# 3DGenomes/TADpole

Measured on NVIDIA B200. Metric: tadpole_calls_per_sec, higher is better.
Workload: dtype f64

## Files before the change

### tadpole_b200/csrc/api.cu

```cuda
#include "common.cuh"
#include <stdarg.h>
#include <algorithm>
#include <mutex>
#include <numeric>
#include <unordered_map>

int tp_sweep_device(tp_ctx *ctx, int min_clusters, int cand_begin, int cand_stride, int *ncand_out);
int tp_ch_device(tp_ctx *ctx, int min_clusters, int ncand, int ld_chs);

static thread_local char g_err[1024] = "";

void tp_set_error(const char *fmt, ...) {
    va_list ap;
    va_start(ap, fmt);
    vsnprintf(g_err, sizeof(g_err), fmt, ap);
    va_end(ap);
}

extern "C" const char *tp_last_error(void) { return g_err; }
extern "C" int tp_version(void) { return 103; }

int tp_pin_reserve(tp_ctx *ctx, size_t bytes) {
    if (bytes <= ctx->pin_cap) return TP_OK;
    if (ctx->pin) cudaFreeHost(ctx->pin);
// ... 57 lines not shown
    }
    TP_ARG(device >= 0 && device < ndev, "tp_ctx_create: device index out of range");
    TP_CUDA(cudaSetDevice(device));
    cudaDeviceProp prop;
    TP_CUDA(cudaGetDeviceProperties(&prop, device));
    if (prop.major < 10) {
        tp_set_error("tp_ctx_create: device %d is sm_%d%d; this library is built for sm_100a (B200) only",
                     device, prop.major, prop.minor);
        return TP_ERR_CUDA;
    }
    tp_ctx *ctx = new tp_ctx();
    ctx->device = device;
    ctx->sm_count = prop.multiProcessorCount;
    ctx->max_smem_optin = (int)prop.sharedMemPerBlockOptin;
    TP_CUDA(cudaStreamCreateWithFlags(&ctx->stream, cudaStreamNonBlocking));
    for (int i = 0; i < EV_COUNT; i++) TP_CUDA(cudaEventCreate(&ctx->ev[i]));
    TP_CUDA(cudaEventCreateWithFlags(&ctx->sync_ev, cudaEventBlockingSync | cudaEventDisableTiming));
    TP_TRY(tp_pin_reserve(ctx, 1 << 16));
    TP_TRY(tp_flags_reset(ctx));
    if (const char *tune = getenv("TADPOLE_TUNE")) {
        std::string t(tune);
        size_t pos = 0;
        while (pos < t.size()) {
            size_t end = t.find(',', pos);
            if (end == std::string::npos) end = t.size();
            const std::string item = t.substr(pos, end - pos);
            pos = end + 1;
            if (item.empty()) continue;
            const size_t eq = item.find('=');
            char *endp = nullptr;
            const double v = eq == std::string::npos ? 0.0 : strtod(item.c_str() + eq + 1, &endp);
            if (eq == std::string::npos || eq == 0 || endp == item.c_str() + eq + 1 || *endp) {
                tp_set_error("tp_ctx_create: TADPOLE_TUNE item '%s' is not key=number", item.c_str());
                tp_ctx_destroy(ctx);
                return TP_ERR_ARG;
            }
            if (tp_ctx_set(ctx, item.substr(0, eq).c_str(), v) != TP_OK) { tp_ctx_destroy(ctx); return TP_ERR_ARG; }
        }
    }
    *out = ctx;
    return TP_OK;
}

extern "C" int tp_ctx_destroy(tp_ctx *ctx) {
    if (!ctx) return TP_OK;
    tp_pool_destroy(ctx);
    tp_group_destroy(ctx);
    cudaSetDevice(ctx->device);
    tp_stream_sync(ctx);
    DevBuf *bufs[] = {&ctx->raw_own, &ctx->rowmean, &ctx->ranks, &ctx->flags, &ctx->qtmp, &ctx->keep, &ctx->X, &ctx->C,
                      &ctx->colstat, &ctx->scores, &ctx->M, &ctx->Y0, &ctx->Y1, &ctx->Y2, &ctx->W, &ctx->G, &ctx->T,
                      &ctx->Q, &ctx->Jw, &ctx->Jv, &ctx->Jt, &ctx->small1, &ctx->small2, &ctx->part, &ctx->resid,
                      &ctx->P, &ctx->Qp, &ctx->d0, &ctx->seqdist, &ctx->order, &ctx->ncl, &ctx->chs, &ctx->bsbuf,
                      &ctx->links, &ctx->harm, &ctx->status, &ctx->islices, &ctx->ioA, &ctx->ioB, &ctx->ioscale, &ctx->lx, &ctx->ly, &ctx->dout, &ctx->dhash, &ctx->lhash,
                      &ctx->itext, &ctx->icounts, &ctx->irows, &ctx->islow, &ctx->icoo, &ctx->raw_next};
    for (DevBuf *b : bufs) b->release();
    tp_comm_destroy_all(ctx);
    for (int i = 0; i < EV_COUNT; i++) if (ctx->ev[i]) cudaEventDestroy(ctx->ev[i]);
    for (cudaEvent_t e : ctx->prof_ev) cudaEventDestroy(e);
    if (ctx->sync_ev) cudaEventDestroy(ctx->sync_ev);
    if (ctx->staged_ev) cudaEventDestroy(ctx->staged_ev);
    for (tp_ctx::UploadLane &ln : ctx->lanes) {
        if (ln.st) { cudaStreamSynchronize(ln.st); cudaStreamDestroy(ln.st); }
        if (ln.done) cudaEventDestroy(ln.done);
        for (int b = 0; b < 2; b++) { if (ln.pin[b]) cudaFreeHost(ln.pin[b]); if (ln.ev[b]) cudaEventDestroy(ln.ev[b]); }
    }
    if (ctx->copy_stream) { cudaStreamSynchronize(ctx->copy_stream); cudaStreamDestroy(ctx->copy_stream); }
    for (int b = 0; b < 2; b++) {
        if (ctx->ipin[b]) cudaFreeHost(ctx->ipin[b]);
        if (ctx->ipin_ev[b]) cudaEventDestroy(ctx->ipin_ev[b]);
    }
    if (ctx->pin) cudaFreeHost(ctx->pin);
    if (ctx->pin_flags) cudaFreeHost(ctx->pin_flags);
    if (ctx->stream) cudaStreamDestroy(ctx->stream);
    delete ctx;
    return TP_OK;
}

extern "C" int tp_ctx_sync(tp_ctx *ctx) {
    TP_ARG(ctx, "tp_ctx_sync: null context");
    for (int r = tp_group_size(ctx) - 1; r >= 0; r--) {
        tp_ctx *m = tp_group_member(ctx, r);
        TP_CUDA(cudaSetDevice(m->device));
        TP_CUDA(tp_stream_sync(m));
    }
    return TP_OK;
}

extern "C" void *tp_ctx_stream(tp_ctx *ctx) { return ctx ? (void *)ctx->stream : nullptr; }
extern "C" long long tp_ctx_launches(tp_ctx *ctx) { return ctx ? ctx->launches : 0; }

extern "C" int tp_ctx_set(tp_ctx *ctx, const char *key, double value) {
    TP_ARG(ctx && key, "tp_ctx_set: null argument");
    if (tp_group_dispatch(ctx)) {
        for (int r = 1; r < tp_group_size(ctx); r++) {
            tp_ctx *m = tp_group_member(ctx, r);
            TpGroup *g = m->group;
            m->group = nullptr;
            const int rc = tp_ctx_set(m, key, value);
            m->group = g;
            TP_TRY(rc);
        }
    }
    std::string k(key);
    if (k == "pca_block") ctx->pca_block = (int)value;
    else if (k == "pca_tol") ctx->pca_tol = value;
    else if (k == "pca_maxit") ctx->pca_maxit = (int)value;
// ... 612 lines not shown
```

### tadpole_b200/csrc/common.cuh

```cuda
#pragma once
#include <cuda_runtime.h>
#include <stdint.h>
#include <stdio.h>
#include <string.h>
#include <math.h>
#include <string>
#include <vector>
#include <functional>
#include "../../include/tadpole_b200.h"

void tp_set_error(const char *fmt, ...);

#define TP_CUDA(call)                                                                     \
    do {                                                                                  \
        cudaError_t e_ = (call);                                                          \
        if (e_ != cudaSuccess) {                                                          \
            tp_set_error("%s:%d: %s -> %s", __FILE__, __LINE__, #call, cudaGetErrorString(e_)); \
            return TP_ERR_CUDA;                                                           \
        }                                                                                 \
    } while (0)

#define TP_TRY(call)                   \
    do {                               \
        int rc_ = (call);              \
// ... 62 lines not shown
    int comm_cur = -1;
    bool comm_grouped = false;
    int last_sweep_ranks = 1;
    int dist_min_n = 4096;
    int igemm_min_n = 1024;
    int iop_min_n = 1024;
    int sync_blocking = 0;
    cudaEvent_t sync_ev = nullptr;
    int shard_sym = 1;
    int mgram_min_n = 1024;
    int iop_final_min_n = 1024;
    int iop_final = 8;
    int io_bn32 = -1;
    double iop_switch = 1e-3;

    int pca_block = 0;
    double pca_tol = 1e-12;
    int pca_maxit = 16;
    int pca_inner = 4;
    int jacobi_direct_max = 512;
    int level_cap = 256;

    DevBuf itext, icounts, irows, islow, icoo;
    void *ipin[2] = {nullptr, nullptr};
    cudaEvent_t ipin_ev[2] = {nullptr, nullptr};
    struct UploadLane { cudaStream_t st = nullptr; void *pin[2] = {nullptr, nullptr}; cudaEvent_t ev[2] = {nullptr, nullptr}; cudaEvent_t done = nullptr; };
    std::vector<UploadLane> lanes;
    int upload_lanes = 4;
    int ingested_n = 0;
    double ingest_stats[4] = {};

    DevBuf raw_own;
    DevBuf raw_next;
    cudaStream_t copy_stream = nullptr;
    cudaEvent_t staged_ev = nullptr;
    const double *staged_mat = nullptr;
    int staged_n = 0, staged_colmajor = 0;
    std::function<void()> after_filter, after_pca;
    const double *raw = nullptr;
    int n = 0;
    int colmajor = 0;
    DevBuf rowmean, ranks, flags, qtmp, keep;
    int nf = 0, ldx = 0;
    DevBuf ioA, ioB, ioscale;
    int io_n = 0;
    bool io_cmax_clean = false;
    DevBuf X, C, colstat, islices;
    bool have_X = false, have_C = false;
    int k = 0, ldk = 0;
    int k_full = 0;
    DevBuf scores, M, Y0, Y1, Y2, W, G, T, Q, Jw, Jv, Jt, small1, small2, part, resid;
    DevBuf status;
    bool have_scores = false;
    DevBuf P, Qp, d0, seqdist, order, ncl, chs, bsbuf, links, harm;
    int ld_chs = 0;
    int last_maxlev = 0;
    std::vector<double> sweep_scores;
    bool have_sweep = false;
    DevBuf lx, ly, dout, dhash, lhash;
    void *pin = nullptr;
    size_t pin_cap = 0;
    int *pin_flags = nullptr;

    double timing[10] = {};
    long lowprec_applications = 0;

    bool prof = false;
    std::vector<cudaEvent_t> prof_ev;
    std::vector<int> prof_cls;
    size_t prof_used = 0;
    double prof_gemm_flop = 0.0;
    double prof_imma_ops = 0.0;
};

enum { PC_ROWMEAN = 0, PC_COMPACT, PC_GEMM, PC_JACOBI, PC_SWEEP, PC_CH, PC_DIFFT, PC_SPARE, PC_CHOL, PC_IGEMM, PC_COMM, PC_SPARE3, PC_ISLICE, PC_SPARE4, PC_SPARE5, PC_SPARE6, PC_COUNT };
void tp_prof_begin(tp_ctx *ctx, int cls);
void tp_prof_end(tp_ctx *ctx);

cudaError_t tp_optin_smem_fn(const void *kernel, const tp_ctx *ctx);
template <class K> static inline cudaError_t tp_optin_smem(K kernel, const tp_ctx *ctx) {
    return tp_optin_smem_fn((const void *)kernel, ctx);
}
int tp_pin_reserve(tp_ctx *ctx, size_t bytes);
cudaError_t tp_stream_sync(tp_ctx *ctx);

static inline int tp_nranks(const tp_ctx *ctx) { return ctx->comm_cur < 0 ? 1 : ctx->comm[ctx->comm_cur].nranks; }
static inline int tp_rank(const tp_ctx *ctx) { return ctx->comm_cur < 0 ? 0 : ctx->comm[ctx->comm_cur].rank; }
struct TpRows { int rpr, r0, r1, padded; };
static inline TpRows tp_rows(const tp_ctx *ctx, int n) {
    const int R = tp_nranks(ctx), rank = tp_rank(ctx);
    TpRows t;
    t.rpr = round_up((n + R - 1) / R, 64);
    t.r0 = rank * t.rpr < n ? rank * t.rpr : n;
    t.r1 = t.r0 + t.rpr < n ? t.r0 + t.rpr : n;
    t.padded = R * t.rpr;
    return t;
}
static inline bool tp_row_sharded(const tp_ctx *ctx, int n) { return tp_nranks(ctx) > 1 && n >= ctx->dist_min_n; }

struct SymShard { int R, rpr; };
__host__ __device__ inline bool ss_need(int i, int j, SymShard s) {
    const int a = i / s.rpr, c = j / s.rpr;
    int d = c - a; if (d < 0) d += s.R;
    if (d == 0) return j >= i;
    if (2 * d < s.R) return true;
    if (2 * d > s.R) return false;
    const int li = i - a * s.rpr, lj = j - c * s.rpr;
// ... 60 lines not shown
```

### tadpole_b200/csrc/coniss.cu

```cuda
#include "common.cuh"

#define INF_D (__longlong_as_double(0x7ff0000000000000LL))

template <bool SMEM, typename T> __device__ __forceinline__ int ld_link(const T *p) { return SMEM ? (int)*p : (int)__ldcg(p); }
template <bool SMEM, typename T> __device__ __forceinline__ void st_link(T *p, int v) { if (SMEM) *p = (T)v; else __stcg(p, (T)v); }

__global__ void rownorm2_kernel(const double *__restrict__ s, int n, int k, int ldk, double *__restrict__ out) {
    int w = (blockIdx.x * blockDim.x + threadIdx.x) >> 5, lane = threadIdx.x & 31;
    if (w >= n) return;
    double a = 0.0;
    for (int c = lane; c < k; c += 32) { double v = s[(size_t)w * ldk + c]; a += v * v; }
    a = warp_sum(a);
    if (lane == 0) out[w] = a;
}

#define PF_CHUNK 128
__global__ void __launch_bounds__(64)
prefix_sums_kernel(const double *__restrict__ s, const double *__restrict__ rn2, int n, int k, int ldk,
                   double *__restrict__ csum) {
    const int c = blockIdx.y * 64 + threadIdx.x, ch = blockIdx.x;
    if (c > ldk) return;
    const int r0 = ch * PF_CHUNK, r1 = min(n, r0 + PF_CHUNK);
    double a0 = 0.0, a1 = 0.0;
    if (c < k) {
        int r = r0;
        for (; r + 1 < r1; r += 2) { a0 += s[(size_t)r * ldk + c]; a1 += s[(size_t)(r + 1) * ldk + c]; }
        if (r < r1) a0 += s[(size_t)r * ldk + c];
    } else if (c == ldk) {
        int r = r0;
        for (; r + 1 < r1; r += 2) { a0 += rn2[r]; a1 += rn2[r + 1]; }
        if (r < r1) a0 += rn2[r];
    }
    csum[(size_t)ch * (ldk + 1) + c] = a0 + a1;
}
__global__ void __launch_bounds__(64)
prefix_write_kernel(const double *__restrict__ s, const double *__restrict__ rn2, const double *__restrict__ csum, int n, int k,
                    int ldk, double *__restrict__ P, double *__restrict__ Qp) {
    const int c = blockIdx.y * 64 + threadIdx.x, ch = blockIdx.x;
    if (c > ldk) return;
    const int r0 = ch * PF_CHUNK, r1 = min(n, r0 + PF_CHUNK);
    double acc = 0.0;
    for (int q = 0; q < ch; q++) acc += csum[(size_t)q * (ldk + 1) + c];
    if (c < k) {
        if (ch == 0) P[c] = 0.0;
        for (int r = r0; r < r1; r++) { acc += s[(size_t)r * ldk + c]; P[(size_t)(r + 1) * ldk + c] = acc; }
    } else if (c < ldk) {
        if (ch == 0) P[c] = 0.0;
        for (int r = r0; r < r1; r++) P[(size_t)(r + 1) * ldk + c] = 0.0;
    } else {
        if (ch == 0) Qp[0] = 0.0;
        for (int r = r0; r < r1; r++) { acc += rn2[r]; Qp[r + 1] = acc; }
    }
}

__global__ void d0_kernel(const double *__restrict__ s, int n, int k, int ldk, double *__restrict__ d0, int ldd) {
    int j = blockIdx.x * blockDim.x + threadIdx.x;
    if (j >= n - 1) return;
    const double *a = s + (size_t)j * ldk, *b = a + ldk;
    double acc = 0.0;
    for (int c = 0; c < k; c++) {
        double t = a[c] - b[c];
        acc += 0.5 * t * t;
        d0[(size_t)c * ldd + j] = acc;
    }
}

__device__ __forceinline__ double lds_f64(unsigned a) { double v; asm volatile("ld.shared.f64 %0, [%1];" : "=d"(v) : "r"(a) : "memory"); return v; }
__device__ __forceinline__ void sts_f64(unsigned a, double v) { asm volatile("st.shared.f64 [%0], %1;" ::"r"(a), "d"(v) : "memory"); }
__device__ __forceinline__ int lds_u16(unsigned a) { unsigned short v; asm volatile("ld.shared.u16 %0, [%1];" : "=h"(v) : "r"(a) : "memory"); return v; }
__device__ __forceinline__ void sts_u16(unsigned a, int v) { asm volatile("st.shared.u16 [%0], %1;" ::"r"(a), "h"((unsigned short)v) : "memory"); }
__device__ __forceinline__ unsigned lds_u32(unsigned a) { unsigned v; asm volatile("ld.shared.u32 %0, [%1];" : "=r"(v) : "r"(a) : "memory"); return v; }
__device__ __forceinline__ void sts_u32(unsigned a, unsigned v) { asm volatile("st.shared.u32 [%0], %1;" ::"r"(a), "r"(v) : "memory"); }
__device__ __forceinline__ int lds_s32(unsigned a) { int v; asm volatile("ld.shared.s32 %0, [%1];" : "=r"(v) : "r"(a) : "memory"); return v; }
__device__ __forceinline__ void sts_s32(unsigned a, int v) { asm volatile("st.shared.s32 [%0], %1;" ::"r"(a), "r"(v) : "memory"); }

template <typename LinkT, bool SMEM> struct Links {
    unsigned sp, sn;
    LinkT *gp, *gn;
    __device__ __forceinline__ int prv(int j) const {
        if (SMEM) return sizeof(LinkT) == 2 ? lds_u16(sp + 2 * j) : lds_s32(sp + 4 * j);
        return (int)__ldcg(gp + j);
    }
    __device__ __forceinline__ int nxt(int j) const {
        if (SMEM) return sizeof(LinkT) == 2 ? lds_u16(sn + 2 * j) : lds_s32(sn + 4 * j);
        return (int)__ldcg(gn + j);
    }
    __device__ __forceinline__ void set_prv(int j, int v) const {
        if (SMEM) { if (sizeof(LinkT) == 2) sts_u16(sp + 2 * j, v); else sts_s32(sp + 4 * j, v); }
        else __stcg(gp + j, (LinkT)v);
    }
    __device__ __forceinline__ void set_nxt(int j, int v) const {
        if (SMEM) { if (sizeof(LinkT) == 2) sts_u16(sn + 2 * j, v); else sts_s32(sn + 4 * j, v); }
        else __stcg(gn + j, (LinkT)v);
    }
};

#define CS_CHUNK 8
#define TIE_REL 1e-11
#define TIE_ABS 1e-24

template <typename LinkT, bool LINKS_SMEM, bool INV_SMEM, bool TRACE>
__global__ void __launch_bounds__(256)
coniss_sweep_kernel(const double *__restrict__ P, int ldk, int n,
                    const double *__restrict__ d0, int ldd,
                    const int *__restrict__ cand_list, int ncand, unsigned cand_smem,
                    double *__restrict__ seqdist, int4 *__restrict__ merges,
                    LinkT *__restrict__ glinks, const double *__restrict__ qtot, long long *__restrict__ trace) {
    extern __shared__ __align__(16) unsigned char smem_raw[];
    const int lane = threadIdx.x & 31, warp = threadIdx.x >> 5, wpc = blockDim.x >> 5;
    const int slot = blockIdx.x * wpc + warp;
    const int n1 = n - 1;
    const int n1p = (n1 + 31) & ~31;
    const int B1 = n1p >> 5;
    const int B1p = (B1 + 31) & ~31;
    const int B2 = B1p >> 5;
    const int B2p = (B2 + 31) & ~31;

    const unsigned sbase0 = (unsigned)__cvta_generic_to_shared(smem_raw);
    const unsigned sinv = sbase0 + (unsigned)wpc * cand_smem;
    if (INV_SMEM) {
        for (int m = threadIdx.x; m <= n; m += blockDim.x) sts_f64(sinv + 8u * m, m ? 1.0 / (double)m : 0.0);
        __syncthreads();
    }
    if (slot >= ncand) return;
    const int cand = cand_list[slot];
    const int ncol = cand + 1;
    const unsigned sbase = sbase0 + (unsigned)warp * cand_smem;
    const unsigned sd = sbase;
    const unsigned sm1 = sd + 8u * n1p;
    const unsigned sm2 = sm1 + 8u * B1p;
    Links<LinkT, true> lk;
    lk.sp = lk.sn = 0; lk.gp = lk.gn = nullptr;
    const unsigned sbits = sm2 + 8u * B2p;
    const int W = (n1 + 31) >> 5;
    if (LINKS_SMEM) { lk.sp = sbits; lk.sn = lk.sp + (unsigned)sizeof(LinkT) * n1; }
    auto bm_prev = [&](int j) -> int {
        for (int w0 = j >> 5; w0 >= 0; w0 -= 32) {
            const int wi = w0 - lane;
            unsigned v = wi >= 0 ? lds_u32(sbits + 4u * wi) : 0u;
            if (wi == (j >> 5)) v &= (1u << (j & 31)) - 1u;
            const unsigned bal = __ballot_sync(0xffffffffu, v != 0u);
            if (bal) {
                const int src = __ffs(bal) - 1;
                return ((w0 - src) << 5) + 31 - __clz(__shfl_sync(0xffffffffu, v, src));
            }
        }
        return -1;
    };
    auto bm_next = [&](int j) -> int {
        for (int w0 = j >> 5; w0 < W; w0 += 32) {
            const int wi = w0 + lane;
            unsigned v = wi < W ? lds_u32(sbits + 4u * wi) : 0u;
            if (wi == (j >> 5)) v &= ~((2u << (j & 31)) - 1u);
            const unsigned bal = __ballot_sync(0xffffffffu, v != 0u);
            if (bal) {
                const int src = __ffs(bal) - 1;
                return ((w0 + src) << 5) + __ffs(__shfl_sync(0xffffffffu, v, src)) - 1;
            }
        }
        return n1;
    };
    const double *d0row = d0 + (size_t)cand * ldd;
    double *seq = seqdist + (size_t)cand * ldd;
    int4 *mrg = merges + (size_t)cand * ldd;

    for (int j = lane; j < n1p; j += 32) sts_f64(sd + 8u * j, (j < n1) ? d0row[j] : INF_D);
    if (LINKS_SMEM) {
        for (int j = lane; j < n1; j += 32) { lk.set_prv(j, j); lk.set_nxt(j, j + 1); }
    } else {
        for (int w = lane; w < W; w += 32)
            sts_u32(sbits + 4u * w, (w << 5) + 32 <= n1 ? 0xffffffffu : ((1u << (n1 - (w << 5))) - 1u));
    }
    for (int b = lane; b < B1p; b += 32) sts_f64(sm1 + 8u * b, INF_D);
    for (int b = lane; b < B2p; b += 32) sts_f64(sm2 + 8u * b, INF_D);
    __syncwarp();
    for (int b = 0; b < B1; b++) {
        double v = warp_min_nonneg(lds_f64(sd + 8u * ((b << 5) + lane)));
        if (lane == 0) sts_f64(sm1 + 8u * b, v);
    }
    __syncwarp();
    for (int b = 0; b < B2; b++) {
        double v = warp_min_nonneg(lds_f64(sm1 + 8u * ((b << 5) + lane)));
        if (lane == 0) sts_f64(sm2 + 8u * b, v);
    }
    __syncwarp();

    auto inv_of = [&](int m) -> double { return INV_SMEM ? lds_f64(sinv + 8u * m) : 1.0 / (double)m; };
    const double tie_abs = TIE_ABS * __ldg(qtot);
    const double *Plane = P + lane;
    double total = 0.0;
    long long tr_acc[6] = {0, 0, 0, 0, 0, 0}, tr_t = 0;
#define CS_TR(ph) do { if (TRACE) { const long long t_ = clock64(); tr_acc[ph] += t_ - tr_t; tr_t = t_; } } while (0)
    for (int t = 0; t < n1; t++) {
        if (TRACE) tr_t = clock64();
        double mn;
        int b2 = 0;
        if (B2p == 32) {
            const double v = lds_f64(sm2 + 8u * lane);
            mn = warp_min_nonneg(v);
            const double thr = fma(mn, TIE_REL, mn) + tie_abs;
            b2 = __ffs(__ballot_sync(0xffffffffu, v <= thr)) - 1;
        } else {
            double v = INF_D;
            for (int q = lane; q < B2p; q += 32) v = fmin(v, lds_f64(sm2 + 8u * q));
            mn = warp_min_nonneg(v);
            const double thr = fma(mn, TIE_REL, mn) + tie_abs;
            for (int q0 = 0; q0 < B2p; q0 += 32) {
                unsigned bal = __ballot_sync(0xffffffffu, lds_f64(sm2 + 8u * (q0 + lane)) <= thr);
                if (bal) { b2 = q0 + __ffs(bal) - 1; break; }
            }
        }
        const double thr = fma(mn, TIE_REL, mn) + tie_abs;
        const unsigned bal1 = __ballot_sync(0xffffffffu, lds_f64(sm1 + 8u * ((b2 << 5) + lane)) <= thr);
        const int b1 = (b2 << 5) + __ffs(bal1) - 1;
        const double leaf = lds_f64(sd + 8u * ((b1 << 5) + lane));
        const unsigned bal0 = __ballot_sync(0xffffffffu, leaf <= thr);
        const int j = (b1 << 5) + __ffs(bal0) - 1;
        mn = __shfl_sync(0xffffffffu, leaf, j & 31);

        CS_TR(0);
        int pj, nj, ppj, nnj;
        if (LINKS_SMEM) {
            pj = lk.prv(j) - 1; nj = lk.nxt(j);
            ppj = pj >= 0 ? lk.prv(pj) - 1 : -1;
            nnj = nj < n1 ? lk.nxt(nj) : n1;
        } else {
            pj = bm_prev(j); nj = bm_next(j);
            ppj = pj >= 0 ? bm_prev(pj) : -1;
            nnj = nj < n1 ? bm_next(nj) : n1;
        }
        const bool hasL = pj >= 0, hasR = nj < n1;
        const int a = ppj + 1, b = pj + 1, c = nj + 1, e = nnj + 1;
        const double *Pa = Plane + (size_t)a * ldk, *Pb = Plane + (size_t)b * ldk;
        const double *Pc = Plane + (size_t)c * ldk, *Pe = Plane + (size_t)e * ldk;
        const int cC = c - b, cLL = b - a, cRR = e - c;
        const double iC = inv_of(cC), iLL = inv_of(cLL), iRR = inv_of(cRR);
        double accL = 0.0, accR = 0.0;
        if (TRACE) { asm volatile("" ::"d"(iC), "d"(iLL), "d"(iRR)); CS_TR(1); }
        for (int c0 = 0; c0 < ncol; c0 += 32 * CS_CHUNK) {
            double va[CS_CHUNK], vb[CS_CHUNK], vc[CS_CHUNK], ve[CS_CHUNK];
#pragma unroll
            for (int u = 0; u < CS_CHUNK; u++) {
                const int col = c0 + 32 * u;
                if (col >= ncol) break;
                const bool ok = col + lane < ncol;
                vb[u] = ok ? __ldg(Pb + col) : 0.0;
                vc[u] = ok ? __ldg(Pc + col) : 0.0;
                va[u] = (ok && hasL) ? __ldg(Pa + col) : 0.0;
                ve[u] = (ok && hasR) ? __ldg(Pe + col) : 0.0;
            }
#pragma unroll
            for (int u = 0; u < CS_CHUNK; u++) {
                if (c0 + 32 * u >= ncol) break;
                const double mC = (vc[u] - vb[u]) * iC;
                const double tL = hasL ? (vb[u] - va[u]) * iLL - mC : 0.0;
                const double tR = hasR ? mC - (ve[u] - vc[u]) * iRR : 0.0;
                accL = fma(tL, tL, accL);
                accR = fma(tR, tR, accR);
            }
        }
        if (TRACE) { asm volatile("" ::"d"(accL), "d"(accR)); CS_TR(2); }
        total += mn;
        if (lane == 0) {
            seq[j] = total;
            mrg[t] = make_int4(j, pj, nj, 0);
        }
#pragma unroll
        for (int o = 16; o > 0; o >>= 1) {
            accL += __shfl_xor_sync(0xffffffffu, accL, o);
            accR += __shfl_xor_sync(0xffffffffu, accR, o);
        }
        accL *= (double)cLL * (double)cC * inv_of(cLL + cC);
        accR *= (double)cC * (double)cRR * inv_of(cC + cRR);

        if (TRACE) { asm volatile("" ::"d"(accL), "d"(accR)); CS_TR(3); }
        if (lane == 0) {
            sts_f64(sd + 8u * j, INF_D);
            if (hasL) { sts_f64(sd + 8u * pj, accL); if (LINKS_SMEM) lk.set_nxt(pj, nj); }
            if (hasR) { sts_f64(sd + 8u * nj, accR); if (LINKS_SMEM) lk.set_prv(nj, pj + 1); }
            if (!LINKS_SMEM) sts_u32(sbits + 4u * (j >> 5), lds_u32(sbits + 4u * (j >> 5)) & ~(1u << (j & 31)));
        }
        __syncwarp();
        const int k0 = j >> 5;
        const int k1 = hasL ? (pj >> 5) : k0;
        const int k2 = hasR ? (nj >> 5) : k0;
        const double x0 = lds_f64(sd + 8u * ((k0 << 5) + lane));
        const double x1 = lds_f64(sd + 8u * ((k1 << 5) + lane));
        const double x2 = lds_f64(sd + 8u * ((k2 << 5) + lane));
        const double r0 = warp_min_nonneg(x0);
        const double r1 = (k1 != k0) ? warp_min_nonneg(x1) : r0;
        const double r2 = (k2 != k0) ? warp_min_nonneg(x2) : r0;
        if (lane == 0) {
            sts_f64(sm1 + 8u * k0, r0);
            if (k1 != k0) sts_f64(sm1 + 8u * k1, r1);
            if (k2 != k0) sts_f64(sm1 + 8u * k2, r2);
        }
        __syncwarp();
        CS_TR(4);
        const int g0 = k0 >> 5, g1 = k1 >> 5, g2 = k2 >> 5;
        const double y0 = warp_min_nonneg(lds_f64(sm1 + 8u * ((g0 << 5) + lane)));
        if (lane == 0) sts_f64(sm2 + 8u * g0, y0);
        if (g1 != g0) {
            const double y1 = warp_min_nonneg(lds_f64(sm1 + 8u * ((g1 << 5) + lane)));
            if (lane == 0) sts_f64(sm2 + 8u * g1, y1);
        }
        if (g2 != g0 && g2 != g1) {
            const double y2 = warp_min_nonneg(lds_f64(sm1 + 8u * ((g2 << 5) + lane)));
            if (lane == 0) sts_f64(sm2 + 8u * g2, y2);
        }
        __syncwarp();
        CS_TR(5);
    }
    if (TRACE && slot == 0 && lane == 0) {
        for (int p = 0; p < 6; p++) trace[p] = tr_acc[p];
        trace[6] = n1;
        trace[7] = ncol;
    }
#undef CS_TR
}

#define CH_WARPS 4
__global__ void __launch_bounds__(32 * CH_WARPS)
ch_kernel(const double *__restrict__ P, const double *__restrict__ Qp, int ldk, int n, int k,
          const double *__restrict__ seqdist, const int4 *__restrict__ merges, int ldd,
          const int *__restrict__ cand_list, int min_clusters,
          double *__restrict__ bs_scratch, int *__restrict__ ncl_out,
          double *__restrict__ chs, int ld_chs) {
    extern __shared__ double s_dl[];
    __shared__ int s_ncl;
    const int tid = threadIdx.x, lane = tid & 31, warp = tid >> 5;
    const int cand = cand_list[blockIdx.x];
    const int n1 = n - 1;
    const double *seq = seqdist + (size_t)cand * ldd;
// ... 71 lines not shown
        ssq = warp_sum(ssq);
    }
    __syncthreads();
    if (tid == 0) {
        const double trS = Qp[n] - ssq / (double)n;
        double W = trS;
        const int mc = min(min_clusters, ncl);
        const double dN = (double)n;
        if (mc <= 1 && ld_chs > 0) out[0] = (dN - 1.0) * (trS - W) / (0.0 * W);
        for (int lev = 2; lev <= nlev; lev++) {
            W -= s_dl[lev];
            if (lev >= mc) out[lev - 1] = (dN - (double)lev) * (trS - W) / ((double)(lev - 1) * W);
        }
    }
}

static int build_cand_list(int k, int begin, int stride, std::vector<int> &out) {
    out.clear();
    for (int c = begin; c < k; c += stride) out.push_back(c);
    for (size_t i = 0, j = out.size(); i + 1 < j; i++, j--) std::swap(out[i], out[j - 1]);
    return (int)out.size();
}

int tp_sweep_device(tp_ctx *ctx, int min_clusters, int cand_begin, int cand_stride, int *ncand_out) {
    TP_ARG(ctx->have_scores, "tp_sweep: no PC scores in the context (run tp_pca or tp_set_scores)");
    TP_ARG(cand_stride >= 1 && cand_begin >= 0, "tp_sweep: bad candidate range");
    TP_ARG(min_clusters >= 1, "tp_sweep: min_clusters must be >= 1");
    const int n = ctx->nf, k = ctx->k, ldk = ctx->ldk;
    TP_ARG(n >= 3, "tp_sweep: need at least 3 bins");
    const int n1 = n - 1;
    const int ldd = round_up(n1, 8);
    std::vector<int> cands;
    const int ncand = build_cand_list(k, cand_begin, cand_stride, cands);
    *ncand_out = ncand;
    cudaStream_t st = ctx->stream;
    if (ncand == 0) {
        TP_TRY(ctx->ncl.reserve((size_t)(2 * k + 8) * sizeof(int)));
        TP_CUDA(cudaMemsetAsync(ctx->ncl.p, 0, k * sizeof(int), st));
        TP_TRY(ctx->seqdist.reserve((size_t)k * ldd * sizeof(double)));
        TP_TRY(ctx->order.reserve((size_t)k * ldd * sizeof(int4)));
        TP_MARK(ctx, EV_SWEEP0);
        TP_MARK(ctx, EV_SWEEP1);
        ctx->have_sweep = true;
        return TP_OK;
    }

    TP_TRY(ctx->P.reserve((size_t)(n + 1) * ldk * sizeof(double)));
    TP_TRY(ctx->Qp.reserve((size_t)(n + 2) * sizeof(double) * 2));
    TP_TRY(ctx->d0.reserve((size_t)k * ldd * sizeof(double)));
    TP_TRY(ctx->seqdist.reserve((size_t)k * ldd * sizeof(double)));
    TP_TRY(ctx->order.reserve((size_t)k * ldd * sizeof(int4)));
    TP_TRY(ctx->ncl.reserve((size_t)(2 * k + 8) * sizeof(int)));
    TP_TRY(ctx->bsbuf.reserve((size_t)ncand * ldd * sizeof(double)));
    int *d_cands = ctx->ncl.as<int>() + k;
    TP_CUDA(cudaMemcpyAsync(d_cands, cands.data(), ncand * sizeof(int), cudaMemcpyHostToDevice, st));
    TP_CUDA(cudaMemsetAsync(ctx->ncl.p, 0, k * sizeof(int), st));

    double *rn2 = ctx->Qp.as<double>() + (n + 2);
    TP_MARK(ctx, EV_SWEEP0);
    rownorm2_kernel<<<(n * 32 + 255) / 256, 256, 0, st>>>(ctx->scores.as<double>(), n, k, ldk, rn2);
    {
        const int nch = (n + PF_CHUNK - 1) / PF_CHUNK;
        TP_TRY(ctx->harm.reserve((size_t)nch * (ldk + 1) * sizeof(double)));
        const dim3 pg(nch, (ldk + 1 + 63) / 64);
        prefix_sums_kernel<<<pg, 64, 0, st>>>(ctx->scores.as<double>(), rn2, n, k, ldk, ctx->harm.as<double>());
        prefix_write_kernel<<<pg, 64, 0, st>>>(ctx->scores.as<double>(), rn2, ctx->harm.as<double>(), n, k, ldk,
                                               ctx->P.as<double>(), ctx->Qp.as<double>());
    }
    d0_kernel<<<(n1 + 127) / 128, 128, 0, st>>>(ctx->scores.as<double>(), n, k, ldk, ctx->d0.as<double>(), ldd);
    ctx->launches += 4;

    const int n1p = round_up(n1, 32), B1p = round_up(n1p / 32, 32), B2p = round_up(B1p / 32, 32);
    const size_t base = (size_t)(n1p + B1p + B2p) * sizeof(double);
    const bool small_links = n <= 65535;
    const size_t link_bytes = round_up((int)((size_t)2 * n1 * (small_links ? 2 : 4)), 8);
    const size_t bitmap_bytes = (size_t)round_up(((n1 + 31) / 32) * 4, 16);
    const size_t inv_bytes = (size_t)(n + 1) * sizeof(double);
    const size_t limit = (size_t)ctx->max_smem_optin;
    TP_ARG(base + bitmap_bytes <= limit, "tp_sweep: matrix too large for the shared-memory dSS array (n > ~28k bins); split by centromere");
    const char *force = getenv("TADPOLE_SWEEP_LINKS");
    bool links_smem = base + link_bytes <= limit;
    if (force && force[0] == 'b') links_smem = false;
    if (force && force[0] == 'a' && base + link_bytes <= limit) links_smem = true;
    const size_t cand_smem = round_up((int)(links_smem ? base + link_bytes : base + bitmap_bytes), 16);
    bool inv_smem = 2 * cand_smem + inv_bytes <= limit;
    const char *e_inv = getenv("TADPOLE_SWEEP_INV"), *e_wpc = getenv("TADPOLE_SWEEP_WPC");
    if (e_inv && e_inv[0] == 'g') inv_smem = false;
    int wpc = (int)((limit - (inv_smem ? inv_bytes : 0)) / cand_smem);
    const int wpc_cap = e_wpc && atoi(e_wpc) > 0 ? atoi(e_wpc) : 4;
    wpc = wpc < 1 ? 1 : (wpc > wpc_cap ? wpc_cap : wpc);
    while (wpc > 1 && (ncand + wpc - 1) / wpc < 16) wpc--;
    const size_t smem = (size_t)wpc * cand_smem + (inv_smem ? inv_bytes : 0);
    const int nblocks = (ncand + wpc - 1) / wpc;
    void *glinks = nullptr;
    long long *trace = nullptr;
    DevBuf trbuf;
    if (getenv("TADPOLE_SWEEP_TRACE")) { TP_TRY(trbuf.reserve(8 * sizeof(long long))); trace = trbuf.as<long long>(); }
#define LAUNCH_SWEEP2(LT, LS, IS, TR)                                                                     \
    do {                                                                                                  \
        TP_CUDA(tp_optin_smem(coniss_sweep_kernel<LT, LS, IS, TR>, ctx)); \
        tp_prof_begin(ctx, PC_SWEEP);                                                                     \
        coniss_sweep_kernel<LT, LS, IS, TR><<<nblocks, 32 * wpc, smem, st>>>(ctx->P.as<double>(), ldk, n, ctx->d0.as<double>(), ldd, \
                                                                 d_cands, ncand, (unsigned)cand_smem, ctx->seqdist.as<double>(), \
                                                                 ctx->order.as<int4>(), (LT *)glinks, ctx->Qp.as<double>() + n, trace); \
        tp_prof_end(ctx);                                                                                 \
    } while (0)
#define LAUNCH_SWEEP(LT, LS, IS) do { if (trace) LAUNCH_SWEEP2(LT, LS, IS, true); else LAUNCH_SWEEP2(LT, LS, IS, false); } while (0)
    if (links_smem) {
        if (small_links) { if (inv_smem) LAUNCH_SWEEP(unsigned short, true, true); else LAUNCH_SWEEP(unsigned short, true, false); }
        else { if (inv_smem) LAUNCH_SWEEP(int, true, true); else LAUNCH_SWEEP(int, true, false); }
    } else {
        if (inv_smem) LAUNCH_SWEEP(unsigned short, false, true); else LAUNCH_SWEEP(unsigned short, false, false);
    }
#undef LAUNCH_SWEEP2
#undef LAUNCH_SWEEP
    ctx->launches += 1;
    TP_CUDA(cudaGetLastError());
    TP_MARK(ctx, EV_SWEEP1);
    if (trace) {
        long long h[8];
        TP_CUDA(cudaStreamSynchronize(st));
        TP_CUDA(cudaMemcpy(h, trace, sizeof(h), cudaMemcpyDeviceToHost));
        static const char *ph[6] = {"find", "links", "p_rows_dot", "reduce_scale", "writeback_l1", "l2"};
        fprintf(stderr, "[sweep trace] n=%d cols=%lld wpc=%d links_smem=%d inv_smem=%d cycles per merge step:", n, h[7], wpc, (int)links_smem, (int)inv_smem);
        for (int p = 0; p < 6; p++) fprintf(stderr, " %s %.0f", ph[p], (double)h[p] / (double)h[6]);
        fprintf(stderr, "\n");
        trbuf.release();
    }
    ctx->have_sweep = true;
    (void)min_clusters;
    return TP_OK;
}

int tp_ch_device(tp_ctx *ctx, int min_clusters, int ncand, int ld_chs) {
    const int n = ctx->nf, k = ctx->k, ldk = ctx->ldk;
    const int ldd = round_up(n - 1, 8);
    cudaStream_t st = ctx->stream;
    TP_TRY(ctx->chs.reserve((size_t)k * ld_chs * sizeof(double)));
    ctx->ld_chs = ld_chs;
    int *d_cands = ctx->ncl.as<int>() + k;
    TP_CUDA(cudaMemsetAsync(ctx->chs.p, 0xff, (size_t)k * ld_chs * sizeof(double), st));
    if (ncand == 0) { TP_MARK(ctx, EV_CH1); return TP_OK; }
    tp_prof_begin(ctx, PC_CH);
    ch_kernel<<<ncand, 32 * CH_WARPS, (size_t)(ld_chs + 2) * sizeof(double), st>>>(ctx->P.as<double>(), ctx->Qp.as<double>(), ldk, n, k,
                                    ctx->seqdist.as<double>(), ctx->order.as<int4>(), ldd, d_cands, min_clusters,
                                    ctx->bsbuf.as<double>(), ctx->ncl.as<int>(), ctx->chs.as<double>(), ld_chs);
    tp_prof_end(ctx);
    ctx->launches += 1;
    TP_CUDA(cudaGetLastError());
    TP_MARK(ctx, EV_CH1);
    return TP_OK;
}
```

Before: 317.6.

## Replace sweep linked lists with warp-parallel bitmap neighbour search and global reciprocal table

Drops the shared-memory prev/next link arrays in the CONISS sweep kernel. Neighbours of a merged cluster are now found from a 32-word window of the alive-bitmap using ballots and shuffles across the warp. The reciprocal table moves from per-block shared memory into a global buffer filled by the rownorm kernel, and the two pair reciprocals are read from it too. Warps per CTA are capped at 3 under a 64 KB per-CTA shared budget so more CTAs can fit per SM. The cost is extra ballot and shuffle work per merge step, plus bm_prev/bm_next fallbacks when a neighbour lies outside the window.

```diff
diff --git a/tadpole_b200/csrc/api.cu b/tadpole_b200/csrc/api.cu
--- a/tadpole_b200/csrc/api.cu
+++ b/tadpole_b200/csrc/api.cu
@@ -133,7 +133,7 @@
                       &ctx->colstat, &ctx->scores, &ctx->M, &ctx->Y0, &ctx->Y1, &ctx->Y2, &ctx->W, &ctx->G, &ctx->T,
                       &ctx->Q, &ctx->Jw, &ctx->Jv, &ctx->Jt, &ctx->small1, &ctx->small2, &ctx->part, &ctx->resid,
                       &ctx->P, &ctx->Qp, &ctx->d0, &ctx->seqdist, &ctx->order, &ctx->ncl, &ctx->chs, &ctx->bsbuf,
-                      &ctx->links, &ctx->harm, &ctx->status, &ctx->islices, &ctx->ioA, &ctx->ioB, &ctx->ioscale, &ctx->lx, &ctx->ly, &ctx->dout, &ctx->dhash, &ctx->lhash,
+                      &ctx->recip, &ctx->harm, &ctx->status, &ctx->islices, &ctx->ioA, &ctx->ioB, &ctx->ioscale, &ctx->lx, &ctx->ly, &ctx->dout, &ctx->dhash, &ctx->lhash,
                       &ctx->itext, &ctx->icounts, &ctx->irows, &ctx->islow, &ctx->icoo, &ctx->raw_next};
     for (DevBuf *b : bufs) b->release();
     tp_comm_destroy_all(ctx);
diff --git a/tadpole_b200/csrc/common.cuh b/tadpole_b200/csrc/common.cuh
--- a/tadpole_b200/csrc/common.cuh
+++ b/tadpole_b200/csrc/common.cuh
@@ -138,7 +138,7 @@
     DevBuf scores, M, Y0, Y1, Y2, W, G, T, Q, Jw, Jv, Jt, small1, small2, part, resid;
     DevBuf status;
     bool have_scores = false;
-    DevBuf P, Qp, d0, seqdist, order, ncl, chs, bsbuf, links, harm;
+    DevBuf P, Qp, d0, seqdist, order, ncl, chs, bsbuf, recip, harm;
     int ld_chs = 0;
     int last_maxlev = 0;
     std::vector<double> sweep_scores;
diff --git a/tadpole_b200/csrc/coniss.cu b/tadpole_b200/csrc/coniss.cu
--- a/tadpole_b200/csrc/coniss.cu
+++ b/tadpole_b200/csrc/coniss.cu
@@ -2,11 +2,11 @@
 
 #define INF_D (__longlong_as_double(0x7ff0000000000000LL))
 
-template <bool SMEM, typename T> __device__ __forceinline__ int ld_link(const T *p) { return SMEM ? (int)*p : (int)__ldcg(p); }
-template <bool SMEM, typename T> __device__ __forceinline__ void st_link(T *p, int v) { if (SMEM) *p = (T)v; else __stcg(p, (T)v); }
-
-__global__ void rownorm2_kernel(const double *__restrict__ s, int n, int k, int ldk, double *__restrict__ out) {
-    int w = (blockIdx.x * blockDim.x + threadIdx.x) >> 5, lane = threadIdx.x & 31;
+__global__ void rownorm2_kernel(const double *__restrict__ s, int n, int k, int ldk, double *__restrict__ out,
+                                double *__restrict__ inv) {
+    const int gid = blockIdx.x * blockDim.x + threadIdx.x;
+    if (gid <= n) inv[gid] = gid ? 1.0 / (double)gid : 0.0;
+    int w = gid >> 5, lane = threadIdx.x & 31;
     if (w >= n) return;
     double a = 0.0;
     for (int c = lane; c < k; c += 32) { double v = s[(size_t)w * ldk + c]; a += v * v; }
@@ -67,48 +67,26 @@
 
 __device__ __forceinline__ double lds_f64(unsigned a) { double v; asm volatile("ld.shared.f64 %0, [%1];" : "=d"(v) : "r"(a) : "memory"); return v; }
 __device__ __forceinline__ void sts_f64(unsigned a, double v) { asm volatile("st.shared.f64 [%0], %1;" ::"r"(a), "d"(v) : "memory"); }
-__device__ __forceinline__ int lds_u16(unsigned a) { unsigned short v; asm volatile("ld.shared.u16 %0, [%1];" : "=h"(v) : "r"(a) : "memory"); return v; }
-__device__ __forceinline__ void sts_u16(unsigned a, int v) { asm volatile("st.shared.u16 [%0], %1;" ::"r"(a), "h"((unsigned short)v) : "memory"); }
 __device__ __forceinline__ unsigned lds_u32(unsigned a) { unsigned v; asm volatile("ld.shared.u32 %0, [%1];" : "=r"(v) : "r"(a) : "memory"); return v; }
 __device__ __forceinline__ void sts_u32(unsigned a, unsigned v) { asm volatile("st.shared.u32 [%0], %1;" ::"r"(a), "r"(v) : "memory"); }
-__device__ __forceinline__ int lds_s32(unsigned a) { int v; asm volatile("ld.shared.s32 %0, [%1];" : "=r"(v) : "r"(a) : "memory"); return v; }
-__device__ __forceinline__ void sts_s32(unsigned a, int v) { asm volatile("st.shared.s32 [%0], %1;" ::"r"(a), "r"(v) : "memory"); }
-
-template <typename LinkT, bool SMEM> struct Links {
-    unsigned sp, sn;
-    LinkT *gp, *gn;
-    __device__ __forceinline__ int prv(int j) const {
-        if (SMEM) return sizeof(LinkT) == 2 ? lds_u16(sp + 2 * j) : lds_s32(sp + 4 * j);
-        return (int)__ldcg(gp + j);
-    }
-    __device__ __forceinline__ int nxt(int j) const {
-        if (SMEM) return sizeof(LinkT) == 2 ? lds_u16(sn + 2 * j) : lds_s32(sn + 4 * j);
-        return (int)__ldcg(gn + j);
-    }
-    __device__ __forceinline__ void set_prv(int j, int v) const {
-        if (SMEM) { if (sizeof(LinkT) == 2) sts_u16(sp + 2 * j, v); else sts_s32(sp + 4 * j, v); }
-        else __stcg(gp + j, (LinkT)v);
-    }
-    __device__ __forceinline__ void set_nxt(int j, int v) const {
-        if (SMEM) { if (sizeof(LinkT) == 2) sts_u16(sn + 2 * j, v); else sts_s32(sn + 4 * j, v); }
-        else __stcg(gn + j, (LinkT)v);
-    }
-};
 
 #define CS_CHUNK 8
 #define TIE_REL 1e-11
 #define TIE_ABS 1e-24
 
-template <typename LinkT, bool LINKS_SMEM, bool INV_SMEM, bool TRACE>
-__global__ void __launch_bounds__(256)
+#define SWEEP_WPC 3
+#define SWEEP_CTA_SMEM (64 << 10)
+template <bool TRACE>
+__global__ void __launch_bounds__(32 * SWEEP_WPC)
 coniss_sweep_kernel(const double *__restrict__ P, int ldk, int n,
                     const double *__restrict__ d0, int ldd,
                     const int *__restrict__ cand_list, int ncand, unsigned cand_smem,
                     double *__restrict__ seqdist, int4 *__restrict__ merges,
-                    LinkT *__restrict__ glinks, const double *__restrict__ qtot, long long *__restrict__ trace) {
+                    const double *__restrict__ inv, const double *__restrict__ qtot, long long *__restrict__ trace) {
     extern __shared__ __align__(16) unsigned char smem_raw[];
     const int lane = threadIdx.x & 31, warp = threadIdx.x >> 5, wpc = blockDim.x >> 5;
     const int slot = blockIdx.x * wpc + warp;
+    if (slot >= ncand) return;
     const int n1 = n - 1;
     const int n1p = (n1 + 31) & ~31;
     const int B1 = n1p >> 5;
@@ -116,24 +94,14 @@
     const int B2 = B1p >> 5;
     const int B2p = (B2 + 31) & ~31;
 
-    const unsigned sbase0 = (unsigned)__cvta_generic_to_shared(smem_raw);
-    const unsigned sinv = sbase0 + (unsigned)wpc * cand_smem;
-    if (INV_SMEM) {
-        for (int m = threadIdx.x; m <= n; m += blockDim.x) sts_f64(sinv + 8u * m, m ? 1.0 / (double)m : 0.0);
-        __syncthreads();
-    }
-    if (slot >= ncand) return;
     const int cand = cand_list[slot];
     const int ncol = cand + 1;
-    const unsigned sbase = sbase0 + (unsigned)warp * cand_smem;
+    const unsigned sbase = (unsigned)__cvta_generic_to_shared(smem_raw) + (unsigned)warp * cand_smem;
     const unsigned sd = sbase;
     const unsigned sm1 = sd + 8u * n1p;
     const unsigned sm2 = sm1 + 8u * B1p;
-    Links<LinkT, true> lk;
-    lk.sp = lk.sn = 0; lk.gp = lk.gn = nullptr;
     const unsigned sbits = sm2 + 8u * B2p;
     const int W = (n1 + 31) >> 5;
-    if (LINKS_SMEM) { lk.sp = sbits; lk.sn = lk.sp + (unsigned)sizeof(LinkT) * n1; }
     auto bm_prev = [&](int j) -> int {
         for (int w0 = j >> 5; w0 >= 0; w0 -= 32) {
             const int wi = w0 - lane;
@@ -160,17 +128,50 @@
         }
         return n1;
     };
+    auto window_word = [&](int wj) -> unsigned {
+        const int wi = wj - 16 + lane;
+        return (wi >= 0 && wi < W) ? lds_u32(sbits + 4u * wi) : 0u;
+    };
+    auto neighbours = [&](int j, unsigned v, int &pj, int &ppj, int &nj, int &nnj) {
+        const int wj = j >> 5, wi = wj - 16 + lane;
+        const unsigned lo = lane < 16 ? v : (lane == 16 ? v & ((1u << (j & 31)) - 1u) : 0u);
+        const unsigned hi = lane > 16 ? v : (lane == 16 ? v & ~((2u << (j & 31)) - 1u) : 0u);
+        const int lo1 = 31 - __clz(lo), hi1 = __ffs(hi) - 1;
+        const unsigned lo_rest = lo & ~(1u << (lo1 & 31)), hi_rest = hi & (hi - 1u);
+        const int lo2 = 31 - __clz(lo_rest), hi2 = __ffs(hi_rest) - 1;
+        const unsigned bl = __ballot_sync(0xffffffffu, lo != 0u), bl2 = __ballot_sync(0xffffffffu, lo_rest != 0u);
+        const unsigned bh = __ballot_sync(0xffffffffu, hi != 0u), bh2 = __ballot_sync(0xffffffffu, hi_rest != 0u);
+        const int sl = 31 - __clz(bl), sh = __ffs(bh) - 1;
+        const int sl2 = ((bl2 >> (sl & 31)) & 1u) ? sl : 31 - __clz(bl & ((1u << (sl & 31)) - 1u));
+        const int sh2 = ((bh2 >> (sh & 31)) & 1u) ? sh : __ffs(bh & ~((2u << (sh & 31)) - 1u)) - 1;
+        const int base = wi << 5;
+        const int p1 = __shfl_sync(0xffffffffu, base + lo1, sl & 31);
+        const int p2 = __shfl_sync(0xffffffffu, base + (lane == sl ? lo2 : lo1), sl2 & 31);
+        const int q1 = __shfl_sync(0xffffffffu, base + hi1, sh & 31);
+        const int q2 = __shfl_sync(0xffffffffu, base + (lane == sh ? hi2 : hi1), sh2 & 31);
+        const bool lo_all = wj - 16 <= 0, hi_all = wj + 15 >= W - 1;
+        if (bl) {
+            pj = p1;
+            ppj = sl2 >= 0 ? p2 : (lo_all ? -1 : bm_prev(pj));
+        } else {
+            pj = lo_all ? -1 : bm_prev(j);
+            ppj = pj >= 0 ? bm_prev(pj) : -1;
+        }
+        if (bh) {
+            nj = q1;
+            nnj = sh2 >= 0 ? q2 : (hi_all ? n1 : bm_next(nj));
+        } else {
+            nj = hi_all ? n1 : bm_next(j);
+            nnj = nj < n1 ? bm_next(nj) : n1;
+        }
+    };
     const double *d0row = d0 + (size_t)cand * ldd;
     double *seq = seqdist + (size_t)cand * ldd;
     int4 *mrg = merges + (size_t)cand * ldd;
 
     for (int j = lane; j < n1p; j += 32) sts_f64(sd + 8u * j, (j < n1) ? d0row[j] : INF_D);
-    if (LINKS_SMEM) {
-        for (int j = lane; j < n1; j += 32) { lk.set_prv(j, j); lk.set_nxt(j, j + 1); }
-    } else {
-        for (int w = lane; w < W; w += 32)
-            sts_u32(sbits + 4u * w, (w << 5) + 32 <= n1 ? 0xffffffffu : ((1u << (n1 - (w << 5))) - 1u));
-    }
+    for (int w = lane; w < W; w += 32)
+        sts_u32(sbits + 4u * w, (w << 5) + 32 <= n1 ? 0xffffffffu : ((1u << (n1 - (w << 5))) - 1u));
     for (int b = lane; b < B1p; b += 32) sts_f64(sm1 + 8u * b, INF_D);
     for (int b = lane; b < B2p; b += 32) sts_f64(sm2 + 8u * b, INF_D);
     __syncwarp();
@@ -185,7 +186,6 @@
     }
     __syncwarp();
 
-    auto inv_of = [&](int m) -> double { return INV_SMEM ? lds_f64(sinv + 8u * m) : 1.0 / (double)m; };
     const double tie_abs = TIE_ABS * __ldg(qtot);
     const double *Plane = P + lane;
     double total = 0.0;
@@ -214,29 +214,23 @@
         const unsigned bal1 = __ballot_sync(0xffffffffu, lds_f64(sm1 + 8u * ((b2 << 5) + lane)) <= thr);
         const int b1 = (b2 << 5) + __ffs(bal1) - 1;
         const double leaf = lds_f64(sd + 8u * ((b1 << 5) + lane));
+        const unsigned win = window_word(b1);
         const unsigned bal0 = __ballot_sync(0xffffffffu, leaf <= thr);
         const int j = (b1 << 5) + __ffs(bal0) - 1;
         mn = __shfl_sync(0xffffffffu, leaf, j & 31);
 
         CS_TR(0);
         int pj, nj, ppj, nnj;
-        if (LINKS_SMEM) {
-            pj = lk.prv(j) - 1; nj = lk.nxt(j);
-            ppj = pj >= 0 ? lk.prv(pj) - 1 : -1;
-            nnj = nj < n1 ? lk.nxt(nj) : n1;
-        } else {
-            pj = bm_prev(j); nj = bm_next(j);
-            ppj = pj >= 0 ? bm_prev(pj) : -1;
-            nnj = nj < n1 ? bm_next(nj) : n1;
-        }
+        neighbours(j, win, pj, ppj, nj, nnj);
+        if (TRACE) { asm volatile("" ::"r"(pj), "r"(ppj), "r"(nj), "r"(nnj)); CS_TR(1); }
         const bool hasL = pj >= 0, hasR = nj < n1;
         const int a = ppj + 1, b = pj + 1, c = nj + 1, e = nnj + 1;
         const double *Pa = Plane + (size_t)a * ldk, *Pb = Plane + (size_t)b * ldk;
         const double *Pc = Plane + (size_t)c * ldk, *Pe = Plane + (size_t)e * ldk;
         const int cC = c - b, cLL = b - a, cRR = e - c;
-        const double iC = inv_of(cC), iLL = inv_of(cLL), iRR = inv_of(cRR);
+        const double iC = __ldg(inv + cC), iLL = __ldg(inv + cLL), iRR = __ldg(inv + cRR);
+        const double iLC = __ldg(inv + cLL + cC), iCR = __ldg(inv + cC + cRR);
         double accL = 0.0, accR = 0.0;
-        if (TRACE) { asm volatile("" ::"d"(iC), "d"(iLL), "d"(iRR)); CS_TR(1); }
         for (int c0 = 0; c0 < ncol; c0 += 32 * CS_CHUNK) {
             double va[CS_CHUNK], vb[CS_CHUNK], vc[CS_CHUNK], ve[CS_CHUNK];
 #pragma unroll
@@ -270,15 +264,15 @@
             accL += __shfl_xor_sync(0xffffffffu, accL, o);
             accR += __shfl_xor_sync(0xffffffffu, accR, o);
         }
-        accL *= (double)cLL * (double)cC * inv_of(cLL + cC);
-        accR *= (double)cC * (double)cRR * inv_of(cC + cRR);
+        accL *= (double)cLL * (double)cC * iLC;
+        accR *= (double)cC * (double)cRR * iCR;
 
         if (TRACE) { asm volatile("" ::"d"(accL), "d"(accR)); CS_TR(3); }
         if (lane == 0) {
             sts_f64(sd + 8u * j, INF_D);
-            if (hasL) { sts_f64(sd + 8u * pj, accL); if (LINKS_SMEM) lk.set_nxt(pj, nj); }
-            if (hasR) { sts_f64(sd + 8u * nj, accR); if (LINKS_SMEM) lk.set_prv(nj, pj + 1); }
-            if (!LINKS_SMEM) sts_u32(sbits + 4u * (j >> 5), lds_u32(sbits + 4u * (j >> 5)) & ~(1u << (j & 31)));
+            if (hasL) sts_f64(sd + 8u * pj, accL);
+            if (hasR) sts_f64(sd + 8u * nj, accR);
+            sts_u32(sbits + 4u * (j >> 5), lds_u32(sbits + 4u * (j >> 5)) & ~(1u << (j & 31)));
         }
         __syncwarp();
         const int k0 = j >> 5;
@@ -456,13 +450,14 @@
     TP_TRY(ctx->order.reserve((size_t)k * ldd * sizeof(int4)));
     TP_TRY(ctx->ncl.reserve((size_t)(2 * k + 8) * sizeof(int)));
     TP_TRY(ctx->bsbuf.reserve((size_t)ncand * ldd * sizeof(double)));
+    TP_TRY(ctx->recip.reserve((size_t)(n + 1) * sizeof(double)));
     int *d_cands = ctx->ncl.as<int>() + k;
     TP_CUDA(cudaMemcpyAsync(d_cands, cands.data(), ncand * sizeof(int), cudaMemcpyHostToDevice, st));
     TP_CUDA(cudaMemsetAsync(ctx->ncl.p, 0, k * sizeof(int), st));
 
     double *rn2 = ctx->Qp.as<double>() + (n + 2);
     TP_MARK(ctx, EV_SWEEP0);
-    rownorm2_kernel<<<(n * 32 + 255) / 256, 256, 0, st>>>(ctx->scores.as<double>(), n, k, ldk, rn2);
+    rownorm2_kernel<<<(n * 32 + 255) / 256, 256, 0, st>>>(ctx->scores.as<double>(), n, k, ldk, rn2, ctx->recip.as<double>());
     {
         const int nch = (n + PF_CHUNK - 1) / PF_CHUNK;
         TP_TRY(ctx->harm.reserve((size_t)nch * (ldk + 1) * sizeof(double)));
@@ -476,47 +471,32 @@
 
     const int n1p = round_up(n1, 32), B1p = round_up(n1p / 32, 32), B2p = round_up(B1p / 32, 32);
     const size_t base = (size_t)(n1p + B1p + B2p) * sizeof(double);
-    const bool small_links = n <= 65535;
-    const size_t link_bytes = round_up((int)((size_t)2 * n1 * (small_links ? 2 : 4)), 8);
     const size_t bitmap_bytes = (size_t)round_up(((n1 + 31) / 32) * 4, 16);
-    const size_t inv_bytes = (size_t)(n + 1) * sizeof(double);
-    const size_t limit = (size_t)ctx->max_smem_optin;
-    TP_ARG(base + bitmap_bytes <= limit, "tp_sweep: matrix too large for the shared-memory dSS array (n > ~28k bins); split by centromere");
-    const char *force = getenv("TADPOLE_SWEEP_LINKS");
-    bool links_smem = base + link_bytes <= limit;
-    if (force && force[0] == 'b') links_smem = false;
-    if (force && force[0] == 'a' && base + link_bytes <= limit) links_smem = true;
-    const size_t cand_smem = round_up((int)(links_smem ? base + link_bytes : base + bitmap_bytes), 16);
-    bool inv_smem = 2 * cand_smem + inv_bytes <= limit;
-    const char *e_inv = getenv("TADPOLE_SWEEP_INV"), *e_wpc = getenv("TADPOLE_SWEEP_WPC");
-    if (e_inv && e_inv[0] == 'g') inv_smem = false;
-    int wpc = (int)((limit - (inv_smem ? inv_bytes : 0)) / cand_smem);
-    const int wpc_cap = e_wpc && atoi(e_wpc) > 0 ? atoi(e_wpc) : 4;
-    wpc = wpc < 1 ? 1 : (wpc > wpc_cap ? wpc_cap : wpc);
+    const size_t cand_smem = round_up((int)(base + bitmap_bytes), 16);
+    TP_ARG(cand_smem <= (size_t)ctx->max_smem_optin,
+           "tp_sweep: matrix too large for the shared-memory dSS array (n > ~28k bins); split by centromere");
+    int wpc = SWEEP_WPC;
+    while (wpc > 1 && wpc * cand_smem > SWEEP_CTA_SMEM) wpc--;
     while (wpc > 1 && (ncand + wpc - 1) / wpc < 16) wpc--;
-    const size_t smem = (size_t)wpc * cand_smem + (inv_smem ? inv_bytes : 0);
+    const size_t smem = (size_t)wpc * cand_smem;
     const int nblocks = (ncand + wpc - 1) / wpc;
-    void *glinks = nullptr;
     long long *trace = nullptr;
     DevBuf trbuf;
     if (getenv("TADPOLE_SWEEP_TRACE")) { TP_TRY(trbuf.reserve(8 * sizeof(long long))); trace = trbuf.as<long long>(); }
-#define LAUNCH_SWEEP2(LT, LS, IS, TR)                                                                     \
+#define LAUNCH_SWEEP(TR)                                                                                  \
     do {                                                                                                  \
-        TP_CUDA(tp_optin_smem(coniss_sweep_kernel<LT, LS, IS, TR>, ctx)); \
+        TP_CUDA(tp_optin_smem(coniss_sweep_kernel<TR>, ctx));                                             \
+         \
+        TP_CUDA(cudaFuncSetAttribute(coniss_sweep_kernel<TR>, cudaFuncAttributePreferredSharedMemoryCarveout,        \
+                                     cudaSharedmemCarveoutMaxShared));                                    \
         tp_prof_begin(ctx, PC_SWEEP);                                                                     \
-        coniss_sweep_kernel<LT, LS, IS, TR><<<nblocks, 32 * wpc, smem, st>>>(ctx->P.as<double>(), ldk, n, ctx->d0.as<double>(), ldd, \
+        coniss_sweep_kernel<TR><<<nblocks, 32 * wpc, smem, st>>>(ctx->P.as<double>(), ldk, n, ctx->d0.as<double>(), ldd, \
                                                                  d_cands, ncand, (unsigned)cand_smem, ctx->seqdist.as<double>(), \
-                                                                 ctx->order.as<int4>(), (LT *)glinks, ctx->Qp.as<double>() + n, trace); \
+                                                                 ctx->order.as<int4>(), ctx->recip.as<double>(), \
+                                                                 ctx->Qp.as<double>() + n, trace);        \
         tp_prof_end(ctx);                                                                                 \
     } while (0)
-#define LAUNCH_SWEEP(LT, LS, IS) do { if (trace) LAUNCH_SWEEP2(LT, LS, IS, true); else LAUNCH_SWEEP2(LT, LS, IS, false); } while (0)
-    if (links_smem) {
-        if (small_links) { if (inv_smem) LAUNCH_SWEEP(unsigned short, true, true); else LAUNCH_SWEEP(unsigned short, true, false); }
-        else { if (inv_smem) LAUNCH_SWEEP(int, true, true); else LAUNCH_SWEEP(int, true, false); }
-    } else {
-        if (inv_smem) LAUNCH_SWEEP(unsigned short, false, true); else LAUNCH_SWEEP(unsigned short, false, false);
-    }
-#undef LAUNCH_SWEEP2
+    if (trace) LAUNCH_SWEEP(true); else LAUNCH_SWEEP(false);
 #undef LAUNCH_SWEEP
     ctx->launches += 1;
     TP_CUDA(cudaGetLastError());
@@ -526,7 +506,7 @@
         TP_CUDA(cudaStreamSynchronize(st));
         TP_CUDA(cudaMemcpy(h, trace, sizeof(h), cudaMemcpyDeviceToHost));
         static const char *ph[6] = {"find", "links", "p_rows_dot", "reduce_scale", "writeback_l1", "l2"};
-        fprintf(stderr, "[sweep trace] n=%d cols=%lld wpc=%d links_smem=%d inv_smem=%d cycles per merge step:", n, h[7], wpc, (int)links_smem, (int)inv_smem);
+        fprintf(stderr, "[sweep trace] n=%d cols=%lld wpc=%d smem/CTA=%zu cycles per merge step:", n, h[7], wpc, smem);
         for (int p = 0; p < 6; p++) fprintf(stderr, " %s %.0f", ph[p], (double)h[p] / (double)h[6]);
         fprintf(stderr, "\n");
         trbuf.release();
```

Result: slower. 304.1 (median of 6 runs) (-4.3%).
